# JialeTao/MRFA

Measured on AMD Instinct MI355X. Metric: frames/sec (256x256 source+driving pair) fwd+bwd, higher is better.
Workload: dtype f32; 1 GPU; vox1.yaml MTIA (TokenPose_B) prior + DenseMotion + RaftFlow refinement, 256x256, bs=8/GPU, fwd+bwd+clip+Adam, train-mode BN, surrogate L1 loss; global_batch=8, parallelism=dp1, prior=mtia, background_predictor=False, sync_bn=False, launch=hipGraph, optimizer=FlatAdam (K20), mfma=bf16x6

## Files before the change

mrfa_amd/csrc/common.h:

```cpp
#pragma once
#include <hip/hip_runtime.h>
#include <stdio.h>
#include <string.h>
#include "mrfa_hip.h"

typedef float f32x16 __attribute__((ext_vector_type(16)));
typedef float f32x4 __attribute__((ext_vector_type(4)));

void mrfa_set_error(const char* fmt, ...);

struct MrfaTuning {
    int conv_small_env;
    int conv_small;
    int conv_halo, conv_halo_min_tiles, conv_halo_pr, conv_halo_phase, conv_halo_bn256, conv_halo_bn192, conv_halo_bn64_fill;
    int conv_lean, conv_lean_min_wgs, conv_lean_geo, gemm_lean;
    int wgrad_halo, wgrad_halo_min_wgs, wgrad_halo_target_wgs, wgrad_halo_phase, wgrad_lean;
    int conv_fewout3, attention_mfma, split_target_256;
};
extern MrfaTuning g_tune;

struct HaloGeo { int PR, BN; bool phase; };

enum class ConvFamily { lean, gemm_lean, small, halo, halo_dgrad, rows_split, rows_f32, refused };
struct ConvPlan {
    ConvFamily family;
    char error[256];
    long long M;
    int KT;
    int lean_geo, gemm_cfg, small_tm, small_tn;
    HaloGeo halo;
    int BM, BN, splitk;
    bool w8;
    bool fused;
    bool fin_in_launch;
    bool reads_w;
    int last_config;
    bool groups_ok, bst_ok, stride2_ok, mask_ok, phase_dgrad_ok;
};
ConvPlan plan_conv(const mrfa_conv_params& p);

enum class WgradFamily { lean, small, halo, tiled, refused };
struct WgradPlan {
    WgradFamily family;
    char error[192];
    long long M;
    bool lean, small;
    bool groups_ok, stride2_ok;
};
WgradPlan plan_wgrad(const mrfa_wgrad_params& p);

int mrfa_conv_split_launch(hipStream_t st, const mrfa_conv_params& p, int KT, long long M, int splitk, int BN);
bool mrfa_conv_halo_eligible(const mrfa_conv_params& p, HaloGeo* geo);
int mrfa_conv_halo_launch(hipStream_t st, const mrfa_conv_params& p, const HaloGeo& geo);
int mrfa_wgrad_split_launch(hipStream_t st, const mrfa_wgrad_params& p, dim3 grid, long long M, long long kps, int tiles_n, int nsplit, int inner,
                            int total_splits, int taps, long long partial_stride, int BM, int BN);

bool mrfa_wgrad_halo_eligible(const mrfa_wgrad_params& p);
int mrfa_wgrad_halo_launch(hipStream_t st, const mrfa_wgrad_params& p);

bool mrfa_fewout3_wgrad(hipStream_t st, const float* x, int ldx, int N, int H, int W, int Cin, const float* dy, int lddy, int Cout, int R, int pad,
                        float* dw, float* dbias, int* rc);

int mrfa_conv_lean_pick(const mrfa_conv_params& p);
int mrfa_conv_lean_launch(hipStream_t st, const mrfa_conv_params& p, int geo);
int mrfa_gemm_lean_pick(const mrfa_conv_params& p, long long M);
int mrfa_gemm_lean_launch(hipStream_t st, const mrfa_conv_params& p, long long M, int cfg);

bool mrfa_conv_small_eligible(const mrfa_conv_params& p, long long M);
int mrfa_conv_small_launch(hipStream_t st, const mrfa_conv_params& p, long long M, int tm, int tn);

// ... 137 lines not shown
```

mrfa_amd/csrc/conv_plan.hip:

```cpp
#include "common.h"
#include <stdarg.h>
#include <stdlib.h>

namespace {
int env_int(const char* name, int dflt) { const char* e = getenv(name); return e ? atoi(e) : dflt; }
int env_on(const char* name) { const char* e = getenv(name); return !(e && e[0] == '0'); }
}

MrfaTuning g_tune = {
     env_on("MRFA_CONV_SMALL"),  1,
     env_on("MRFA_CONV_HALO"),  128,  0,  1,  1,
     1,  1,
     env_on("MRFA_CONV_LEAN"),  128,  -1,
     env_int("MRFA_GEMM_LEAN", 1),
     env_on("MRFA_WGRAD_HALO"),  192,  256,  1,
     env_on("MRFA_WGRAD_LEAN"),
     1,  env_on("MRFA_ATTENTION_MFMA"),  env_int("MRFA_SPLIT_TARGET_256", 1),
};

enum TuneKind { T_ON, T_INT, T_NONNEG, T_NONNEG_ON, T_LEVEL, T_POS };
static const struct { const char* key; int* field; TuneKind kind; } TUNING_KEYS[] = {
    {"conv_small", &g_tune.conv_small, T_ON},
    {"conv_halo", &g_tune.conv_halo, T_ON},
    {"conv_halo_min_tiles", &g_tune.conv_halo_min_tiles, T_INT},
    {"conv_halo_pr", &g_tune.conv_halo_pr, T_INT},
    {"conv_halo_phase", &g_tune.conv_halo_phase, T_ON},
    {"conv_halo_bn256", &g_tune.conv_halo_bn256, T_ON},
    {"conv_halo_bn192", &g_tune.conv_halo_bn192, T_ON},
    {"conv_halo_bn64_fill", &g_tune.conv_halo_bn64_fill, T_ON},
    {"conv_lean", &g_tune.conv_lean, T_ON},
    {"conv_lean_min_wgs", &g_tune.conv_lean_min_wgs, T_NONNEG},
    {"conv_lean_geo", &g_tune.conv_lean_geo, T_INT},
    {"gemm_lean", &g_tune.gemm_lean, T_LEVEL},
    {"wgrad_halo", &g_tune.wgrad_halo, T_ON},
    {"wgrad_halo_min_wgs", &g_tune.wgrad_halo_min_wgs, T_NONNEG},
    {"wgrad_halo_target_wgs", &g_tune.wgrad_halo_target_wgs, T_POS},
    {"wgrad_halo_phase", &g_tune.wgrad_halo_phase, T_NONNEG_ON},
    {"wgrad_lean", &g_tune.wgrad_lean, T_ON},
    {"conv_fewout3", &g_tune.conv_fewout3, T_ON},
    {"attention_mfma", &g_tune.attention_mfma, T_ON},
};

extern "C" int mrfa_set_tuning(const char* key, int value) {
    if (!key) return -1;
    for (const auto& k : TUNING_KEYS) {
        if (strcmp(key, k.key)) continue;
        const int prev = *k.field;
        switch (k.kind) {
            case T_ON: *k.field = value != 0; break;
            case T_INT: *k.field = value; break;
            case T_NONNEG: if (value >= 0) *k.field = value; break;
            case T_NONNEG_ON: if (value >= 0) *k.field = value != 0; break;
            case T_LEVEL: if (value >= 0) *k.field = value > 2 ? 2 : value; break;
            case T_POS: if (value > 0) *k.field = value; break;
        }
        return prev;
    }
    return -1;
}

namespace {
constexpr int BK = 32;

template <typename Plan>
Plan& refuse(Plan& c, const char* fmt, ...) {
    va_list ap;
    va_start(ap, fmt);
    vsnprintf(c.error, sizeof(c.error), fmt, ap);
    va_end(ap);
    c.family = decltype(c.family)::refused;
    return c;
}

void plan_rows(ConvPlan& c, const mrfa_conv_params& p, int mode) {
    const bool flat = p.kflat > 0;
    const long long M = c.M;
    const int KT = c.KT;
    const int nb = p.nbatch > 1 ? p.nbatch : 1;
    int BN = 128;
    {
        const int cands[4] = {128, 96, 64, 32};
        const double pen[4] = {1.0, 1.08, 1.16, 1.3};
        double best = 1e18;
        for (int i = 0; i < 4; ++i) {
            if (cands[i] == 96 && flat) continue;
            const double cost = (double)cdiv(p.Cout, cands[i]) * cands[i] * pen[i];
            if (cost < best) { best = cost; BN = cands[i]; }
        }
    }
    if (mode >= 1 && !flat && p.Cout >= 32) BN = p.Cout <= 64 ? 64 : 128;
    auto ntiles = [&](int bm, int bn) { return ((M + bm - 1) / bm) * cdiv(p.Cout, bn) * nb; };
    int BM = 128;
    if (BN == 96 && ntiles(128, 96) < 384) BN = 128;
// ... 164 lines not shown
```

mrfa_amd/csrc/sample.hip:

```cpp
#include "mfma_bf16.h"

namespace {

struct Taps {
    int x0, y0;
    float fx, fy;
};

__device__ __forceinline__ Taps make_taps(float ix, float iy) {
    Taps t;
    const float fx0 = floorf(ix), fy0 = floorf(iy);
    t.x0 = (int)fx0;
    t.y0 = (int)fy0;
    t.fx = ix - fx0;
    t.fy = iy - fy0;
    return t;
}


struct Taps4 {
    size_t o00, o01, o10, o11;
    float w00, w01, w10, w11;
    float fx, fy;
    bool ok00, ok01, ok10, ok11;
// ... 291 lines not shown
__global__ void resize_bwd_kernel(const float* __restrict__ dout, int lddo, int N, int Hi, int Wi, int C, float* __restrict__ din,
                                  int lddi, int Ho, int Wo, float mul, long long total) {
    for (long long i = blockIdx.x * (long long)blockDim.x + threadIdx.x; i < total; i += (long long)gridDim.x * blockDim.x) {
        const long long opix = i / C;
        const int c = (int)(i - opix * C);
        const int ox = (int)(opix % Wo);
        const long long t = opix / Wo;
        const int oy = (int)(t % Ho);
        const long long n = t / Ho;
        int x0, x1, y0, y1;
        float fx, fy;
        resize_src(ox, Wi, Wo, x0, x1, fx);
        resize_src(oy, Hi, Ho, y0, y1, fy);
        const float g = dout[(size_t)opix * lddo + c] * mul;
        float* b = din + (size_t)n * Hi * Wi * lddi + c;
        atomicAdd(b + ((size_t)y0 * Wi + x0) * lddi, g * (1.f - fx) * (1.f - fy));
        atomicAdd(b + ((size_t)y0 * Wi + x1) * lddi, g * fx * (1.f - fy));
        atomicAdd(b + ((size_t)y1 * Wi + x0) * lddi, g * (1.f - fx) * fy);
        atomicAdd(b + ((size_t)y1 * Wi + x1) * lddi, g * fx * fy);
    }
}

__global__ void resize_bwd_gather_kernel(const float* __restrict__ dout, int lddo, int N, int Hi, int Wi, int C, float* __restrict__ din,
                                         int lddi, int Ho, int Wo, float mul, long long total) {
    const float sy = Ho > 1 ? (float)(Hi - 1) / (float)(Ho - 1) : 0.f, sx = Wo > 1 ? (float)(Wi - 1) / (float)(Wo - 1) : 0.f;
    for (long long i = blockIdx.x * (long long)blockDim.x + threadIdx.x; i < total; i += (long long)gridDim.x * blockDim.x) {
        const long long ipix = i / C;
        const int c = (int)(i - ipix * C);
        const int ix = (int)(ipix % Wi);
        const long long t = ipix / Wi;
        const int iy = (int)(t % Hi);
        const long long n = t / Hi;
        int oy_lo = sy > 0.f ? (int)floorf((float)(iy - 1) / sy) - 1 : 0, oy_hi = sy > 0.f ? (int)ceilf((float)(iy + 1) / sy) + 1 : Ho - 1;
        int ox_lo = sx > 0.f ? (int)floorf((float)(ix - 1) / sx) - 1 : 0, ox_hi = sx > 0.f ? (int)ceilf((float)(ix + 1) / sx) + 1 : Wo - 1;
        oy_lo = max(oy_lo, 0); oy_hi = min(oy_hi, Ho - 1); ox_lo = max(ox_lo, 0); ox_hi = min(ox_hi, Wo - 1);
        const float* g = dout + (size_t)n * Ho * Wo * lddo + c;
        float acc = 0.f;
        for (int oy = oy_lo; oy <= oy_hi; ++oy) {
            int y0, y1; float fy;
            resize_src(oy, Hi, Ho, y0, y1, fy);
            const float wy = (y0 == iy ? 1.f - fy : 0.f) + (y1 == iy ? fy : 0.f);
            if (wy == 0.f) continue;
            float row = 0.f;
            for (int ox = ox_lo; ox <= ox_hi; ++ox) {
                int x0, x1; float fx;
                resize_src(ox, Wi, Wo, x0, x1, fx);
                const float wx = (x0 == ix ? 1.f - fx : 0.f) + (x1 == ix ? fx : 0.f);
                if (wx != 0.f) row += wx * g[((size_t)oy * Wo + ox) * lddo];
            }
            acc += wy * row;
        }
        din[(size_t)ipix * lddi + c] += acc * mul;
    }
}

struct ResizeSumArgs {
    int n;
    int prefix[MRFA_RESIZE_SUM_MAX + 1];
    mrfa_resize_sum_desc d[MRFA_RESIZE_SUM_MAX];
};

template <bool BWD>
__global__ __launch_bounds__(256) void resize_sum_multi_kernel(const ResizeSumArgs a) {
    int lo = 0, hi = a.n;
    while (hi - lo > 1) {
        const int mid = (lo + hi) >> 1;
        if ((int)blockIdx.x >= a.prefix[mid]) lo = mid; else hi = mid;
    }
    const mrfa_resize_sum_desc& d = a.d[lo];
    const long long i = (long long)((int)blockIdx.x - a.prefix[lo]) * 256 + threadIdx.x;
    const long long total = (long long)d.N * d.Hd * d.Wd * d.C;
    if (i >= total) return;
    const long long pix = i / d.C;
    const int c = (int)(i - pix * d.C);
    const int px = (int)(pix % d.Wd);
    const long long t = pix / d.Wd;
    const int py = (int)(t % d.Hd);
    const long long n = t / d.Hd;
    float* dst = d.dst + (size_t)pix * d.ldd + c;
    float v = d.overwrite ? 0.f : *dst;
    bool first = d.overwrite != 0;
    for (int k = 0; k < d.nterm; ++k) {
        const float* __restrict__ src = d.term[k].src;
        const int lds = d.term[k].lds, Hs = d.term[k].Hs, Ws = d.term[k].Ws;
        const float mul = d.term[k].mul;
        float r;
        if (Hs == d.Hd && Ws == d.Wd) {
            r = src[(size_t)pix * lds + c] * mul;
        } else if (!BWD) {
            int x0, x1, y0, y1;
            float fx, fy;
            resize_src(px, Ws, d.Wd, x0, x1, fx);
            resize_src(py, Hs, d.Hd, y0, y1, fy);
            const float* b = src + (size_t)n * Hs * Ws * lds + c;
            const float top = b[((size_t)y0 * Ws + x0) * lds] * (1.f - fx) + b[((size_t)y0 * Ws + x1) * lds] * fx;
            const float bot = b[((size_t)y1 * Ws + x0) * lds] * (1.f - fx) + b[((size_t)y1 * Ws + x1) * lds] * fx;
            r = (top * (1.f - fy) + bot * fy) * mul;
        } else {
            const int Hi = d.Hd, Wi = d.Wd, Ho = Hs, Wo = Ws;
            const float sy = Ho > 1 ? (float)(Hi - 1) / (float)(Ho - 1) : 0.f, sx = Wo > 1 ? (float)(Wi - 1) / (float)(Wo - 1) : 0.f;
            int oy_lo = sy > 0.f ? (int)floorf((float)(py - 1) / sy) - 1 : 0, oy_hi = sy > 0.f ? (int)ceilf((float)(py + 1) / sy) + 1 : Ho - 1;
            int ox_lo = sx > 0.f ? (int)floorf((float)(px - 1) / sx) - 1 : 0, ox_hi = sx > 0.f ? (int)ceilf((float)(px + 1) / sx) + 1 : Wo - 1;
            oy_lo = max(oy_lo, 0); oy_hi = min(oy_hi, Ho - 1); ox_lo = max(ox_lo, 0); ox_hi = min(ox_hi, Wo - 1);
            const float* g = src + (size_t)n * Ho * Wo * lds + c;
            float acc = 0.f;
            for (int oy = oy_lo; oy <= oy_hi; ++oy) {
// ... 218 lines not shown
                       in_rep, Hi, Wi, C, grid, ldg, N, Ho, Wo, out, ldo, mode, total);
    MRFA_CHECK_LAUNCH("grid_sample_fwd");
    return 0;
}

extern "C" int mrfa_grid_sample_bf16_fwd(void* stream, const unsigned short* in, int ldi, long long in_bstride, int in_rep, int Hi, int Wi, int C,
                                         const float* grid, int ldg, int N, int Ho, int Wo, float* out, int ldo, int mode) {
    MRFA_CHECK_ARG(in && grid && out && C > 0 && N > 0 && in_rep >= 1 && Hi > 0 && Wi > 0 && Ho > 0 && Wo > 0 && ldi >= C && ldo >= C && ldg >= 2 &&
                   (mode == 0 || mode == 1), "grid_sample_bf16_fwd: bad args");
    MRFA_CHECK_ARG(C % 8 == 0 && ldi % 8 == 0 && in_bstride % 8 == 0 && ldo % 4 == 0 && aligned16(in) && aligned16(out),
                   "grid_sample_bf16_fwd: needs C %% 8 == 0, ldi %% 8 == 0, in_bstride %% 8 == 0, ldo %% 4 == 0 and 16-byte aligned in / out "
                   "(C %d, ldi %d, ldo %d)", C, ldi, ldo);
    const long long npix = (long long)N * Ho * Wo;
    const int c8 = C / 8;
    const int lpp = c8 % 64 == 0 ? 64 : (c8 == 32 ? 32 : (c8 == 16 ? 16 : (c8 == 8 ? 8 : 1)));
    dim3 g(stream_grid(npix * c8, 256));
#define GSH(L) hipLaunchKernelGGL((grid_sample_bf16_fwd_kernel<L>), g, dim3(256), 0, (hipStream_t)stream, in, ldi, in_bstride, in_rep, Hi, Wi, C, \
                                   grid, ldg, npix, Ho, Wo, out, ldo, mode)
    if (lpp == 64) GSH(64); else if (lpp == 32) GSH(32); else if (lpp == 16) GSH(16); else if (lpp == 8) GSH(8); else GSH(1);
#undef GSH
    MRFA_CHECK_LAUNCH("grid_sample_bf16_fwd");
    return 0;
}

extern "C" int mrfa_grid_sample_bwd(void* stream, const float* in, int ldi, long long in_bstride, int in_rep, int Hi, int Wi, int C,
                                    const float* grid, int ldg, int N, int Ho, int Wo, const float* dout, int lddo, int mode,
                                    float* din, int lddi, long long din_bstride, float* dgrid, int lddg) {
    MRFA_CHECK_ARG(in && grid && dout && C > 0 && N > 0 && in_rep >= 1 && Hi > 0 && Wi > 0 && Ho > 0 && Wo > 0 && ldi >= C && lddo >= C && ldg >= 2 &&
                   (!din || lddi >= C) && (!dgrid || lddg >= 2) && (mode == 0 || mode == 1),
                   "grid_sample_bwd: bad args (sizes must be positive, ldi >= C, lddo >= C, ldg >= 2, lddi >= C with din, lddg >= 2 with dgrid, mode 0 or 1; "
                   "C %d, ldi %d, lddo %d, ldg %d, lddi %d, lddg %d, mode %d)", C, ldi, lddo, ldg, lddi, lddg, mode);
    const long long npix = (long long)N * Ho * Wo;
    const int lpp = C % 256 == 0 ? 64 : (C == 128 ? 32 : (C == 64 ? 16 : 0));
    if (lpp && !din && ldi % 4 == 0 && lddo % 4 == 0 && in_bstride % 4 == 0 && aligned16(in) && aligned16(dout)) {
        dim3 g(stream_grid(npix * C / 4, 256));
#define GSB(L) hipLaunchKernelGGL((grid_sample_bwd_vec_kernel<L>), g, dim3(256), 0, (hipStream_t)stream, in, ldi, in_bstride, in_rep, Hi, Wi, C, \
                                   grid, ldg, npix, Ho, Wo, dout, lddo, mode, din, lddi, din_bstride, dgrid, lddg)
        if (lpp == 64) GSB(64); else if (lpp == 32) GSB(32); else GSB(16);
#undef GSB
        MRFA_CHECK_LAUNCH("grid_sample_bwd(vec)");
        return 0;
    }
    const long long waves = (long long)N * Ho * cdiv(Wo, GS_RUN) * cdiv(C, 64);
    hipLaunchKernelGGL(grid_sample_bwd_kernel, dim3(stream_grid(waves * 64, 256)), dim3(256), 0, (hipStream_t)stream, in, ldi, in_bstride,
                       in_rep, Hi, Wi, C, grid, ldg, npix, Ho, Wo, dout, lddo, mode, din, lddi, din_bstride, dgrid, lddg);
    MRFA_CHECK_LAUNCH("grid_sample_bwd");
    return 0;
}

extern "C" int mrfa_resize_bilinear_fwd(void* stream, const float* in, int ldi, int N, int Hi, int Wi, int C, float* out, int ldo,
                                        int Ho, int Wo, float scale_mul, int accumulate) {
    MRFA_CHECK_ARG(in && out && C > 0 && N > 0 && Hi > 0 && Wi > 0 && Ho > 0 && Wo > 0 && ldi >= C && ldo >= C,
                   "resize_fwd: bad args (sizes must be positive, ldi >= C, ldo >= C; C %d, ldi %d, ldo %d, %d x %d -> %d x %d)", C, ldi, ldo, Hi, Wi, Ho, Wo);
    const long long total = (long long)N * Ho * Wo * C;
    hipLaunchKernelGGL(resize_fwd_kernel, dim3(stream_grid(total, 256)), dim3(256), 0, (hipStream_t)stream, in, ldi, N, Hi, Wi, C, out, ldo,
                       Ho, Wo, scale_mul, accumulate, total);
    MRFA_CHECK_LAUNCH("resize_fwd");
    return 0;
}

extern "C" int mrfa_resize_bilinear_bwd(void* stream, const float* dout, int lddo, int N, int Hi, int Wi, int C, float* din, int lddi,
                                        int Ho, int Wo, float scale_mul) {
    MRFA_CHECK_ARG(dout && din && C > 0 && N > 0 && Hi > 0 && Wi > 0 && Ho > 0 && Wo > 0 && lddo >= C && lddi >= C,
                   "resize_bwd: bad args (sizes must be positive, lddo >= C, lddi >= C; C %d, lddo %d, lddi %d, %d x %d -> %d x %d)", C, lddo, lddi, Hi, Wi, Ho, Wo);
    if (Ho >= Hi && Wo >= Wi) {
        const long long total_in = (long long)N * Hi * Wi * C;
        hipLaunchKernelGGL(resize_bwd_gather_kernel, dim3(stream_grid(total_in, 256)), dim3(256), 0, (hipStream_t)stream, dout, lddo, N, Hi,
                           Wi, C, din, lddi, Ho, Wo, scale_mul, total_in);
        MRFA_CHECK_LAUNCH("resize_bwd_gather");
        return 0;
    }
    const long long total = (long long)N * Ho * Wo * C;
    hipLaunchKernelGGL(resize_bwd_kernel, dim3(stream_grid(total, 256)), dim3(256), 0, (hipStream_t)stream, dout, lddo, N, Hi, Wi, C, din,
                       lddi, Ho, Wo, scale_mul, total);
    MRFA_CHECK_LAUNCH("resize_bwd");
    return 0;
}

static int resize_sum_launch(void* stream, const mrfa_resize_sum_desc* descs, int n, bool bwd, const char* what) {
    MRFA_CHECK_ARG(n >= 0 && (n == 0 || descs), "%s: bad args", what);
    for (int base = 0; base < n; base += MRFA_RESIZE_SUM_MAX) {
        ResizeSumArgs a;
        a.n = n - base < MRFA_RESIZE_SUM_MAX ? n - base : MRFA_RESIZE_SUM_MAX;
        int blocks = 0;
        for (int i = 0; i < a.n; ++i) {
            const mrfa_resize_sum_desc& d = descs[base + i];
            MRFA_CHECK_ARG(d.dst && d.N > 0 && d.Hd > 0 && d.Wd > 0 && d.C > 0 && d.nterm >= 1 && d.nterm <= MRFA_RESIZE_SUM_TERMS, "%s: record %d: bad sizes / term count", what, base + i);
            for (int k = 0; k < d.nterm; ++k) {
                MRFA_CHECK_ARG(d.term[k].src && d.term[k].Hs > 0 && d.term[k].Ws > 0, "%s: record %d term %d: null source / bad size", what, base + i, k);
                if (bwd) MRFA_CHECK_ARG(d.term[k].Hs >= d.Hd && d.term[k].Ws >= d.Wd, "%s: record %d term %d: the backward takes up-sampling (or same-size) terms only", what, base + i, k);
            }
            a.d[i] = d;
            a.prefix[i] = blocks;
            const long long total = (long long)d.N * d.Hd * d.Wd * d.C;
            MRFA_CHECK_ARG(total < (1ll << 31) - 256 && blocks + (total + 255) / 256 < (1ll << 30), "%s: record %d too large", what, base + i);
            blocks += (int)((total + 255) / 256);
        }
        a.prefix[a.n] = blocks;
        if (bwd) hipLaunchKernelGGL((resize_sum_multi_kernel<true>), dim3(blocks), dim3(256), 0, (hipStream_t)stream, a);
        else hipLaunchKernelGGL((resize_sum_multi_kernel<false>), dim3(blocks), dim3(256), 0, (hipStream_t)stream, a);
        MRFA_CHECK_LAUNCH(what);
    }
    return 0;
}

extern "C" int mrfa_resize_sum_multi(void* stream, const mrfa_resize_sum_desc* descs, int n) {
    return resize_sum_launch(stream, descs, n, false, "resize_sum_multi");
}

extern "C" int mrfa_resize_sum_multi_bwd(void* stream, const mrfa_resize_sum_desc* descs, int n) {
    return resize_sum_launch(stream, descs, n, true, "resize_sum_multi_bwd");
}

extern "C" int mrfa_corr_lookup_fwd(void* stream, const float* vol0, const float* vol1, int Hs, int Ws, const float* coords, int ldc,
                                    long long Q, int radius, float* out, int ldo) {
    MRFA_CHECK_ARG(radius >= 0 && radius <= 3, "corr_lookup: window must fit one wave (0 <= radius <= 3, got %d)", radius);
    MRFA_CHECK_ARG(vol0 && vol1 && coords && out && Q > 0 && Hs >= 2 && Ws >= 2 && ldc >= 2 && ldo >= 2 * (2 * radius + 1) * (2 * radius + 1),
                   "corr_lookup_fwd: bad args (Hs, Ws >= 2, ldc >= 2, ldo >= 2 (2r+1)^2; Hs %d, Ws %d, ldc %d, ldo %d, radius %d)", Hs, Ws, ldc, ldo, radius);
// ... 57 lines not shown
```

mrfa_amd/engine.py:

```python
from __future__ import annotations

import contextlib
import os

import ctypes as C
from typing import Callable, List, NamedTuple, Optional, Sequence

import torch

from . import hip

BN_EPS = 1e-5
FORCE_TILE = 0
BN_MOMENTUM = 0.1
CAPTURE_KEY = 0
DIRECT_PARAM_GRADS = False
WGRAD_STREAM = False


class Marks:

    def __init__(self, dev, n: int = 256):
        self.buf = torch.zeros(n, dtype=torch.int64, device=dev)
        self.names: List[str] = []
# ... 206 lines not shown

STAT_GROUPS = 1
METRICS_TILE = (32, 32)


class FrameTile(NamedTuple):
    src: torch.Tensor
    y0: int = 0
    x0: int = 0
    kp: Optional[torch.Tensor] = None
    radius: float = 0.0
    colors: Optional[torch.Tensor] = None
    border: bool = False


class stat_groups:

    def __init__(self, groups: int):
        self.groups = int(groups)

    def __enter__(self):
        global STAT_GROUPS
        self.prev, STAT_GROUPS = STAT_GROUPS, self.groups

    def __exit__(self, *exc):
        global STAT_GROUPS
        STAT_GROUPS = self.prev
        return False


class direct_param_grads:
    def __enter__(self):
        global DIRECT_PARAM_GRADS
        self.prev, DIRECT_PARAM_GRADS = DIRECT_PARAM_GRADS, True

    def __exit__(self, *exc):
        global DIRECT_PARAM_GRADS
        DIRECT_PARAM_GRADS = self.prev


def _direct_ok(*params) -> bool:
    return DIRECT_PARAM_GRADS and all(p is None or (p.grad is not None and p.grad.is_contiguous() and p.grad.dtype == torch.float32)
                                      for p in params)


def _r4(c: int) -> int:
    return (c + 3) // 4 * 4


def _up(c: int, m: int) -> int:
    return (c + m - 1) // m * m


def _conv_params() -> hip.ConvParams:
    p = hip.ConvParams()
    p.tile = FORCE_TILE
    return p


class Storage:
    __slots__ = ("data", "dtype", "grad", "rows", "ld", "grad_noinit", "fresh", "bwd_masked", "bn_hint", "seq", "plan")

    def __init__(self, data: torch.Tensor):
        assert data.dim() == 2 and data.dtype in (torch.float32, torch.bfloat16) and data.is_contiguous()
        self.data = data
        self.dtype = data.dtype
        self.rows, self.ld = data.shape
        self.grad: Optional[torch.Tensor] = None
        self.grad_noinit = False
        self.fresh = False
        self.bwd_masked = False
        self.bn_hint = None
        self.seq = -1
        self.plan = None

    def grad_buf(self) -> torch.Tensor:
        if self.dtype != torch.float32:
            raise TypeError("a bf16 storage has no gradient buffer (bf16 activations are inference caches)")
        if self.grad is None:
            self.grad = torch.zeros_like(self.data)
        elif self.fresh:
            self.grad.zero_()
            self.fresh = False
            if self.plan is not None and self.seq >= 0:
                self.plan.add(self.seq)
        return self.grad


class View:
    __slots__ = ("st", "N", "H", "W", "C", "coff", "zpad")

    def __init__(self, st: Storage, N: int, H: int, W: int, C_: int, coff: int = 0, zpad: bool = False):
        assert N * H * W == st.rows and coff + C_ <= st.ld, (N, H, W, C_, coff, st.rows, st.ld)
        self.st, self.N, self.H, self.W, self.C, self.coff = st, N, H, W, C_, coff
        self.zpad = zpad

    @property
    def rows(self) -> int:
        return self.st.rows

    @property
    def ld(self) -> int:
        return self.st.ld

    @property
    def dtype(self) -> torch.dtype:
# ... 478 lines not shown

    def _register(self, st: "Storage"):
        st.seq, st.plan = len(self.storages), self.zero_plan
        self.storages.append(st)

    def wrap_nhwc(self, t: torch.Tensor) -> View:
        assert t.dim() == 4 and t.is_contiguous() and t.dtype == torch.float32
        N, H, W, C_ = t.shape
        return View(Storage(t.view(N * H * W, C_)), N, H, W, C_)

    def from_nchw(self, t: torch.Tensor, out: Optional[View] = None) -> View:
        N, C_, H, W = t.shape
        t = t.contiguous().float()
        out = out or self.new(N, H, W, C_)
        self._chk(self.L.mrfa_nchw_to_nhwc(self.s, t.data_ptr(), out.ptr, out.ld, N, C_, H, W, 0), "nchw_to_nhwc")
        return out

    def to_nchw(self, v: View) -> torch.Tensor:
        t = torch.empty((v.N, v.C, v.H, v.W), dtype=torch.float32, device=self.dev)
        self._chk(self.L.mrfa_nhwc_to_nchw(self.s, v.ptr, v.ld, t.data_ptr(), v.N, v.C, v.H, v.W, 0), "nhwc_to_nchw")
        return t

    def to_bf16(self, v: View) -> View:
        if self.record:
            raise RuntimeError("Ctx.to_bf16: bf16 activations are inference caches, not legal in a recording (training) program")
        out = View(Storage(torch.empty((v.rows, v.C), dtype=torch.bfloat16, device=self.dev)), v.N, v.H, v.W, v.C)
        self._chk(self.L.mrfa_cast_bf16(self.s, v.ptr, v.ld, v.rows, v.C, out.ptr16, out.ld), "cast_bf16")
        return out

    def grad_to_nchw(self, v: View) -> torch.Tensor:
        t = torch.empty((v.N, v.C, v.H, v.W), dtype=torch.float32, device=self.dev)
        self._chk(self.L.mrfa_nhwc_to_nchw(self.s, v.gptr, v.ld, t.data_ptr(), v.N, v.C, v.H, v.W, 0), "nhwc_to_nchw(grad)")
        return t

    def seed_grad_nchw(self, v: View, g: torch.Tensor):
        g = g.contiguous().float()
        self._chk(self.L.mrfa_nchw_to_nhwc(self.s, g.data_ptr(), v.gptr, v.ld, v.N, v.C, v.H, v.W, 1), "seed grad")

    def f32(self, n, zero=False):
        return (torch.zeros if zero else torch.empty)(n, dtype=torch.float32, device=self.dev)

    def f64z(self, n):
        return self.pool64.take(n)

    @staticmethod
    def _claim(v: View) -> bool:
        st = v.st
        if st.grad is not None and st.fresh and v.coff == 0 and v.C == st.ld:
            st.fresh = False
            return True
        return False

    def conv(self, x: View, conv: torch.nn.Conv2d, out: Optional[View] = None, *, relu=False, ups=False, pre=None,
             stats: Optional[torch.Tensor] = None, res: Optional[View] = None, need_dx=True, use_bias=True, relu_in=False, fin=None) -> View:
        cw = convw(conv)
        relu_in = bool(relu_in and RELU_IN and self.record and need_dx and pre is None and not ups)
        if relu_in:
            assert x.coff == 0 and x.C == x.st.ld, "relu_in: the view must cover its storage (every producer skips its ReLU backward)"
            x.st.bwd_masked = True
        assert x.C == cw.Cin, (x.C, cw.Cin)
        Hv, Wv = (x.H * 2, x.W * 2) if ups else (x.H, x.W)
        Ho, Wo = Hv + 2 * cw.pad - cw.R + 1, Wv + 2 * cw.pad - cw.S + 1
        assert out is None or (out.N, out.H, out.W, out.C) == (x.N, Ho, Wo, cw.Cout)
        bias = conv.bias if use_bias else None
        direct = (cw.fewout and not ups and pre is None and res is None and stats is None and not relu
                  and x.ld % 4 == 0 and x.coff % 4 == 0)
        if direct:
            out = out or self.new(x.N, Ho, Wo, cw.Cout)
            self._chk(self.L.mrfa_conv_fewout_fwd(self.s, x.ptr, x.ld, x.N, x.H, x.W, cw.Cin, cw.layout("fewout").data_ptr(),
                                                  bias.data_ptr() if bias is not None else None, out.ptr, out.ld, cw.Cout, cw.R, cw.pad, 0),
                      "conv_fewout_fwd")
            if self.record:
                def bwd_direct():
                    if not out.has_grad:
                        return
                    dw, db = cw.grad_acc(self.pool32)
                    dyp = out.gptr

                    def launch():
                        self._chk(self.L.mrfa_conv_fewout_wgrad(hip.stream_ptr(), x.ptr, x.ld, x.N, x.H, x.W, cw.Cin, dyp, out.ld, cw.Cout, cw.R,
                                                                cw.pad, dw.data_ptr(), db.data_ptr() if (bias is not None and db is not None) else None),
                                  "conv_fewout_wgrad")
                    if self._defer_ok(cw):
                        self.wdefer.add(launch)
                    else:
                        launch()
                    if need_dx:
                        self._conv_dgrad(x, cw, out, ups, pre, relu_in)
                self.tape.append(bwd_direct)
                self._touch(cw)
            return out
        p = _conv_params()
        p.x, p.ldx, p.Hin, p.Win, p.ups, p.N, p.Cin = x.ptr, x.ld, x.H, x.W, int(ups), x.N, cw.Cin
        padded = cw.fwd_flat and x.zpad and x.coff % 4 == 0 and pre is None
        fp32 = self._weight_fields(p, cw, "fwd", padded)
        if self.split and not cw.fwd_flat and ups and cw.R == 3 and cw.S == 3 and cw.pad == 1 and PHASE_UPCONV:
            wph = cw.layout("fwd_phase")
            p.w_phase, p.w_phase_piece = wph.data_ptr(), wph.numel() // 3
        p.Cout, p.Hout, p.Wout = cw.Cout, Ho, Wo
        p.R, p.S, p.pad = cw.R, cw.S, cw.pad
        if pre is not None:
            p.in_scale, p.in_shift, p.in_relu = pre[0].data_ptr(), pre[1].data_ptr(), 1
            if self.train and self.groups > 1:
                p.groups = self.groups
        p.bias = bias.data_ptr() if bias is not None else None
        p.relu = int(relu)
        if res is not None:
            p.res, p.ldr = res.ptr, res.ld
        p.alpha, p.nbatch = 1.0, 1
        if stats is not None:
            p.stats, p.groups = stats.data_ptr(), self.groups
        out = self._conv_out(p, out, x.N, Ho, Wo, cw.Cout)
        late_stats = self._stats_or_late(p, stats, fin, out.rows, pre)
        self._fp32_weights(p, fp32)
        self._launch_conv(p, "conv2d", cw.Cin)
        if late_stats:
            self._bn_stats_into(out, stats)

        if self.record:
            def bwd():
                if not out.has_grad:
                    return
                if relu and not out.st.bwd_masked:
                    self._chk(self.L.mrfa_act_bwd(self.s, out.ptr, out.ld, out.gptr, out.ld, out.rows, out.C, 1, out.gptr, out.ld, 0),
                              "relu_bwd")
                if res is not None:
                    self._chk(self.L.mrfa_copy_view(self.s, out.gptr, out.ld, out.rows, out.C, res.gptr, res.ld, 1.0, 1), "res_bwd")
                if conv.weight.requires_grad:
                    self._conv_wgrad(x, cw, out, ups, pre, bias is not None)
                if need_dx:
                    self._conv_dgrad(x, cw, out, ups, pre, relu_in)
            self.tape.append(bwd)
            self._touch(cw)
        return out

    def _weight_fields(self, p, cw: ConvW, gemm: str, padded: bool = False, planes: bool = True, query: Optional[int] = None):
        g = cw.gemms[gemm]
        rows, k32 = _up(g.rows, 128), _up(g.K, 32)
        if g.flat and not padded:
            p.w_ld, p.w_tap, p.kflat = _up(cw.T * g.K, 32), 0, cw.T * g.K
            p.ktab = g.ktab().data_ptr()
        else:
            p.Cin = k32
            p.w_ld, p.w_tap, p.kflat = k32, rows * k32, 0
            if planes and (self.split or self.bf16):
                p.w_piece = 0 if self.bf16 else cw.T * rows * k32
                p.w_split = query or cw.layout(gemm + ("_rne" if self.bf16 else "_split")).data_ptr()
        p.w_rows = rows
        fp32 = lambda: cw.layout(gemm, padded)
        p.w = query or p.w_split or fp32().data_ptr()
        return fp32

    def _stats_or_late(self, p, stats, fin, rows: int, pre=None) -> bool:
        if stats is None:
            return False
        if self.groups > 1 and not self.L.mrfa_conv2d_groups_supported(C.byref(p)):
            assert pre is None, "a prologue with statistic groups where the library has none: ask prologue_ok() first"
            p.stats, p.groups = None, 0
            return True
        if fin is not None:
            self._fin_params(p, fin, stats, rows)
        return False

    @staticmethod
    def _wgrad_params(x: View, cw: ConvW, dy: int, ldy: int, Ho: int, Wo: int, dw: int, ups=False, stride: int = 0, pre=None) -> hip.WgradParams:
        q = hip.WgradParams()
        q.x, q.ldx, q.Hin, q.Win, q.ups, q.N, q.Cin = x.ptr, x.ld, x.H, x.W, int(ups), x.N, cw.Cin
        if pre is not None:
            q.in_scale, q.in_shift, q.in_relu, q.groups = pre[0], pre[1], 1, pre[2]
        q.dy, q.ldy, q.Cout, q.Hout, q.Wout = dy, ldy, cw.Cout, Ho, Wo
        q.R, q.S, q.pad, q.stride = cw.R, cw.S, cw.pad, stride
        q.dw, q.alpha, q.nbatch, q.ksplit = dw, 1.0, 1, 0
        return q

    def _fp32_weights(self, p, pack):
        ph = p.w_split or p.w_phase
        if not ph or p.w != ph:
            return
        if not (LAZY_FP32_PACKS and not self.L.mrfa_conv2d_reads_fp32_weights(C.byref(p))):
            p.w = pack().data_ptr()

    def _conv_out(self, p, out: Optional[View], N, Ho, Wo, Cout) -> View:
        rows = N * Ho * Wo
        if FUSED_SPLITK and rows <= 32768:
# ... 1213 lines not shown
```

mrfa_amd/modules/raft.py:

```python
from __future__ import annotations

import functools
import math
from typing import List

import torch
import torch.nn.functional as F
from torch import nn

from ..engine import Ctx, Storage, View, run_program
from .generator import OcclusionAwareGenerator
from .util import _FN, Hourglass, batch_bilinear_sampler, bilinear_sampler, coords_grid, coords_grid_nhwc, kp2gaussian


class CorrBlock:

    def __init__(self, corr, num_levels=2, radius=3):
        if num_levels != 2:
            raise NotImplementedError("CorrBlock: the lookup kernel holds the reference's two pyramid levels (raft.py:238)")
        assert corr.dim() == 4 and corr.shape[1] == 1 and corr.shape[2] % 2 == 0 and corr.shape[3] % 2 == 0
        self.num_levels, self.radius = num_levels, radius
        self.corr = corr

    def __call__(self, coords):
        corr, r = self.corr, self.radius
        BQ, _, H, W = corr.shape
        B, _, h1, w1 = coords.shape
        assert B * h1 * w1 == BQ, "CorrBlock: one source map per query pixel"

        def program(e: Ctx, corr_, coords_):
            vol0 = corr_.contiguous().float().view(BQ, H * W)
            vol1 = torch.empty((BQ, (H // 2) * (W // 2)), dtype=torch.float32, device=vol0.device)
            e._chk(e.L.mrfa_avgpool2_fwd(e.s, vol0.data_ptr(), 1, BQ, H, W, 1, vol1.data_ptr(), 1), "corr pyramid level 1")
            cv = e.wrap_nhwc(coords_.float().permute(0, 2, 3, 1).contiguous())
            d = {}

            def dvols():
                if not d:
                    d[0], d[1] = torch.zeros_like(vol0), torch.zeros_like(vol1)
                return d[0], d[1]
            o = e.corr_lookup(vol0, vol1, dvols, H, W, cv, radius=r)

            def dcorr():
                if not d:
                    return None
                e._chk(e.L.mrfa_unpool2_acc(e.s, d[1].data_ptr(), 1, BQ, H // 2, W // 2, 1, d[0].data_ptr(), 1, 0.25), "corr pyramid bwd")
                return d[0].view(BQ, 1, H, W)
            return (e.to_nchw(o),), (lambda g: e.seed_grad_nchw(o, g),), \
                (dcorr, (lambda: cv.st.grad.view(B, h1, w1, 2).permute(0, 3, 1, 2) if cv.has_grad else None))
        return run_program(_FN, program, [corr, coords])[0]


class BasicMotionEncoder(nn.Module):

    def __init__(self, num_levels=2, radius=3):
        super().__init__()
        cor_planes = num_levels * (2 * radius + 1) ** 2
        self.convc1 = nn.Conv2d(cor_planes, 128, 1, padding=0)
        self.convc2 = nn.Conv2d(128, 96, 3, padding=1)
        self.convf1 = nn.Conv2d(2, 128, 7, padding=3)
        self.convf2 = nn.Conv2d(128, 64, 3, padding=1)
        self.conv = nn.Conv2d(64 + 96, 128 - 2, 3, padding=1)

    def run(self, e: Ctx, flow: View, corr: View, out: View):
        cor1 = e.conv(corr, self.convc1, relu=True)
        corflo = e.new(flow.N, flow.H, flow.W, 160)
        e.conv(cor1, self.convc2, out=corflo.slice(0, 96), relu=True, relu_in=True)
        flo1 = e.conv(flow, self.convf1, relu=True)
        e.conv(flo1, self.convf2, out=corflo.slice(96, 160), relu=True, relu_in=True)
        e.conv(corflo, self.conv, out=out.slice(0, 126), relu=True, relu_in=True)
        e.copy(flow, out=out.slice(126, 128))

    def forward(self, delta_flow, corr):
        def program(e: Ctx, flow_, corr_):
            fv = e.from_nchw(flow_)
            cv = e.from_nchw(corr_, out=e.new(corr_.shape[0], corr_.shape[2], corr_.shape[3], corr_.shape[1], pad32=True))
            out = e.new(fv.N, fv.H, fv.W, 128)
            self.run(e, fv, cv, out)
            return (e.to_nchw(out),), (lambda g: e.seed_grad_nchw(out, g),), \
                ((lambda: e.grad_to_nchw(fv) if fv.has_grad else None), (lambda: e.grad_to_nchw(cv) if cv.has_grad else None))
        return run_program(self, program, [delta_flow, corr])[0]


class RefineFlow(nn.Module):

    def __init__(self):
        super().__init__()
        self.convc1 = nn.Conv2d(192, 128, 3, padding=1)
        self.conv1 = nn.Conv2d(256, 128, 3, padding=1)
        self.conv2 = nn.Conv2d(128, 2, 3, padding=1)
        self.convo1 = nn.Conv2d(256, 128, 3, padding=1)
        self.convo2 = nn.Conv2d(128, 1, 3, padding=1)

    def run(self, e: Ctx, inp: View, ctx: View, ctx_relu=False) -> View:
        e.conv(ctx, self.convc1, out=inp.slice(128, 256), relu=True, relu_in=ctx_relu)
        h1 = e.conv(inp, self.conv1, relu=True)
        d = e.new(inp.N, inp.H, inp.W, 3)
        e.conv(h1, self.conv2, out=d.slice(0, 2), relu_in=True)
        h2 = e.conv(inp, self.convo1, relu=True)
        e.conv(h2, self.convo2, out=d.slice(2, 3), relu_in=True)
        return d

    def forward(self, m_f, warp_f):
        def program(e: Ctx, mf_, wf_):
            inp = e.new(mf_.shape[0], mf_.shape[2], mf_.shape[3], 256)
            mv = e.from_nchw(mf_, out=inp.slice(0, 128))
            wv = e.from_nchw(wf_)
            d = self.run(e, inp, wv)
            return (e.to_nchw(d), e.to_nchw(inp)), ((lambda g: e.seed_grad_nchw(d, g)), (lambda g: e.seed_grad_nchw(inp, g))), \
                ((lambda: e.grad_to_nchw(mv) if mv.has_grad else None), (lambda: e.grad_to_nchw(wv) if wv.has_grad else None))
        out, inp = run_program(self, program, [m_f, warp_f])
        return out, inp


class _CorrVolume:

    def __init__(self, e: Ctx, q: View, k: View, kpool: View, scale: float):
        self.e, self.q, self.k, self.kp, self.scale = e, q, k, kpool, scale
        B, Q, S0, S1, D = q.N, q.H * q.W, k.H * k.W, kpool.H * kpool.W, q.C
        self.B, self.Q, self.S0, self.S1, self.D = B, Q, S0, S1, D
        Bs = k.N
        T = B // Bs
        assert Bs * T == B and kpool.N == Bs, "_CorrVolume: the frames of every source, consecutive"
        if T > 1 and e.record:
# ... 139 lines not shown
            outs = (e.to_nchw(out), e.to_nchw(warp_img), self._strip(e, occs))
            seed = ((lambda g: e.seed_grad_nchw(out, g)), (lambda g: e.seed_grad_nchw(warp_img, g)), None)
            return outs, seed, in_grads

        pos = self.pos_embedding

        in_d = e.kp_gaussian(kp_d, 0.1, e.new(b, h, w, kp_d.shape[1]), pos=pos)
        if cache is not None:
            k_s, k_pool = cache["k_s"], cache["k_pool"]
            fe_d = self.kp.run(e, in_d)
            q_d = e.conv(fe_d, self.kp_head)
        else:
            in_s = self._source_input(e, kp_s, img, h, w)
            k_s = e.conv(self.kp_img.run(e, in_s), self.kp_img_head)
            k_pool = e.avgpool2(k_s)
            fe_d = self.kp.run(e, in_d)
            q_d = e.conv(fe_d, self.kp_head)
        in_grads = ((lambda: e.ext_grads.get(id(kp_s))), (lambda: e.ext_grads.get(id(kp_d)))) + in_grads[2:]
        base = self.basic_res_index
        q_levels = {base: q_d}
        for i in range(base - 1, -1, -1):
            q_levels[i] = e.avgpool2(q_levels[i + 1])
        vols = {i: _CorrVolume(e, q_levels[i], k_s, k_pool, self.scale) for i in range(base + 1)} if corr == "volume" else None

        with e.fused_resizes():
            init_flow = e.copy(deform, mul=(h - 1) / 2.0)
            e.copy(_grid_const(e, b, h, w, -1.0, (h - 1) / 2.0, img_full), out=init_flow, acc=True, nograd=True)
        r0 = size // 32
        with e.fused_resizes():
            flow = e.resize(init_flow, r0, r0, mul=1.0 / 8.0)
            occ = e.resize(prior_occ, r0, r0)

        lv_c = gen.level_channels()
        cats = [e.new(b, r0 * (2 ** i), r0 * (2 ** i), 2 * lv_c[i]) for i in range(gen.num_up_blocks)]

        out_warp_f, out_occ = [], []
        d_f_pre = d_occ_pre = None
        for i in range(self.total_iter):
            r = r0 * (2 ** i)
            f = feature[i]
            if i < base:
                cscale, lv, rq = float(2 ** (base - i)), i, r
                flow_q = flow
            else:
                cscale, lv, rq = 1.0, base, h
                flow_q = e.resize(flow, h, w, mul=0.5 ** (i - base)) if i > base else flow
            with e.fused_resizes():
                coords = e.copy(flow_q, mul=cscale)
                e.copy(_grid_const(e, b, rq, rq, cscale, 0.0, img_full), out=coords, acc=True, nograd=True)
            if vols is not None:
                cfeat = e.corr_lookup(vols[lv].vol0, vols[lv].vol1, vols[lv].dvols, h, w, coords)
            else:
                cfeat = e.corr_direct(q_levels[lv], k_s, k_pool, coords, self.scale, k_rep=T)
            if i > base:
                cfeat = e.resize(cfeat, r, r)
            inp = e.new(b, r, r, 256)
            self.corr_enc.run(e, flow, cfeat, inp)
            ctx = e.grid_sample(f, flow, 1, in_rep=T)
            ctx = e.conv(ctx, self.to_context[i], relu=True)
            d_flow = self.refine.run(e, inp, ctx, ctx_relu=True)
            grid_c = None
            with e.fused_resizes():
                flow_w = e.copy(flow)
                e.copy(d_flow.slice(0, 2), out=flow_w, acc=True)
                occ_new = e.copy(occ)
                e.copy(d_flow.slice(2, 3), out=occ_new, acc=True)
                if i < gen.num_up_blocks:
                    grid_c = e.resize(deform, r, r) if i != base else deform
                if i < self.num_iter - 1:
                    r2 = r * 2
                    sc = 2 ** (base - i) / 2.0
                    nflow = e.resize(d_flow.slice(0, 2), r2, r2, mul=2.0)
                    e.resize(init_flow, r2, r2, mul=1.0 / sc, out=nflow, acc=True)
                    nocc = e.resize(d_flow.slice(2, 3), r2, r2)
                    e.resize(prior_occ, r2, r2, out=nocc, acc=True)
                    if i == 0:
                        d_f_pre = e.resize(d_flow.slice(0, 2), r2, r2, mul=2.0)
                        d_occ_pre = e.resize(d_flow.slice(2, 3), r2, r2)
                    else:
                        e.resize(d_f_pre, r2, r2, mul=2.0, out=nflow, acc=True)
                        e.resize(d_occ_pre, r2, r2, out=nocc, acc=True)
                        nd = e.resize(d_flow.slice(0, 2), r2, r2, mul=2.0)
                        e.resize(d_f_pre, r2, r2, mul=2.0, out=nd, acc=True)
                        no = e.resize(d_flow.slice(2, 3), r2, r2)
                        e.resize(d_occ_pre, r2, r2, out=no, acc=True)
                        d_f_pre, d_occ_pre = nd, no
            out_warp_f.append(e.grid_sample(f, flow_w, 1, in_rep=T))
            out_occ.append(e.act(occ_new, 2))
            if i < gen.num_up_blocks:
                e.grid_sample(f, grid_c, 0, out=cats[i].slice(lv_c[i], 2 * lv_c[i]), in_rep=T)
            if i < self.num_iter - 1:
                flow, occ = nflow, nocc
        warp_img = e.grid_sample(imgf, flow, 1, in_rep=T, need_din=False)
        out = gen.run_decode(e, out_warp_f, warp_img, out_occ, cats)
        strip = self._strip(e, out_occ + [e.act(prior_occ, 2)])
        outs = (e.to_nchw(out), e.to_nchw(warp_img), strip)
        seed = ((lambda g: e.seed_grad_nchw(out, g)), (lambda g: e.seed_grad_nchw(warp_img, g)), None)
        return outs, seed, in_grads

    def forward(self, kp_s, kp_d, dense_motion, img, img_full, source_cache=None, corr="volume"):
        if check_corr(corr) == "direct":
            if self.training:
                raise ValueError('corr="direct" is an inference mode (the direct correlation kernel has no backward): call eval() first, training keeps the volumes')
            ins_grad = (kp_s, kp_d, dense_motion['deformation'], dense_motion['occlusion'])
            if torch.is_grad_enabled() and any(t.requires_grad for t in (*self.parameters(), *ins_grad)):
                raise ValueError('corr="direct" has no backward: run it under torch.no_grad() (gradients are enabled and a parameter or input requires one)')
        bs = source_cache["shape"][0] if source_cache is not None else img_full.shape[0]
        b = dense_motion['deformation'].shape[0]
        if b != bs:
            if source_cache is None:
# ... 18 lines not shown
```

Baseline: 101.8 pairs/s.

## Apply 1x1 corr conv before upsampling and add vectorized resize kernels

For refinement levels above base, the 1x1 convc1 now runs on the low-resolution correlation features and its pre-activation output is bilinearly upsampled, with the ReLU applied as a prologue of convc2. Because both the 1x1 conv and bilinear resize are linear, this commutes and cuts the 1x1 conv work and the resize channel count. Separately, float4-vectorized resize forward and gather-backward kernels are added behind a tuning flag. The risks are that the bias now passes through the resize (bilinear weights sum to one, so it is preserved), the ReLU prologue path uses identity scale/shift vectors, and the backward masking must be handled through the new relu_pro flag.

```diff
diff --git a/mrfa_amd/csrc/common.h b/mrfa_amd/csrc/common.h
--- a/mrfa_amd/csrc/common.h
+++ b/mrfa_amd/csrc/common.h
@@ -16,6 +16,7 @@
     int conv_lean, conv_lean_min_wgs, conv_lean_geo, gemm_lean;
     int wgrad_halo, wgrad_halo_min_wgs, wgrad_halo_target_wgs, wgrad_halo_phase, wgrad_lean;
     int conv_fewout3, attention_mfma, split_target_256;
+    int resize_vec;
 };
 extern MrfaTuning g_tune;
 
diff --git a/mrfa_amd/csrc/conv_plan.hip b/mrfa_amd/csrc/conv_plan.hip
--- a/mrfa_amd/csrc/conv_plan.hip
+++ b/mrfa_amd/csrc/conv_plan.hip
@@ -16,6 +16,7 @@
      env_on("MRFA_WGRAD_HALO"),  192,  256,  1,
      env_on("MRFA_WGRAD_LEAN"),
      1,  env_on("MRFA_ATTENTION_MFMA"),  env_int("MRFA_SPLIT_TARGET_256", 1),
+     1,
 };
 
 enum TuneKind { T_ON, T_INT, T_NONNEG, T_NONNEG_ON, T_LEVEL, T_POS };
@@ -39,6 +40,7 @@
     {"wgrad_lean", &g_tune.wgrad_lean, T_ON},
     {"conv_fewout3", &g_tune.conv_fewout3, T_ON},
     {"attention_mfma", &g_tune.attention_mfma, T_ON},
+    {"resize_vec", &g_tune.resize_vec, T_ON},
 };
 
 extern "C" int mrfa_set_tuning(const char* key, int value) {
diff --git a/mrfa_amd/csrc/sample.hip b/mrfa_amd/csrc/sample.hip
--- a/mrfa_amd/csrc/sample.hip
+++ b/mrfa_amd/csrc/sample.hip
@@ -367,6 +367,108 @@
         }
         din[(size_t)ipix * lddi + c] += acc * mul;
     }
+}
+
+struct ResizeVecGeo { int lg, C4, cpr, units; };
+
+__global__ __launch_bounds__(256) void resize_fwd_vec_kernel(const float* __restrict__ in, int ldi, int Hi, int Wi, float* __restrict__ out, int ldo,
+                                                             int Ho, int Wo, float mul, int acc, ResizeVecGeo g) {
+    for (int u = blockIdx.x; u < g.units; u += gridDim.x) {
+        const int row = u / g.cpr;
+        const int j = (u - row * g.cpr) * 256 + (int)threadIdx.x;
+        const int ox = j >> g.lg, q = j & ((1 << g.lg) - 1);
+        if (ox >= Wo || q >= g.C4) continue;
+        const int n = row / Ho, oy = row - n * Ho;
+        int x0, x1, y0, y1;
+        float fx, fy;
+        resize_src(ox, Wi, Wo, x0, x1, fx);
+        resize_src(oy, Hi, Ho, y0, y1, fy);
+        const float* b = in + (size_t)n * Hi * Wi * ldi + 4 * q;
+        const f32x4 v00 = *(const f32x4*)(b + ((size_t)y0 * Wi + x0) * ldi), v01 = *(const f32x4*)(b + ((size_t)y0 * Wi + x1) * ldi);
+        const f32x4 v10 = *(const f32x4*)(b + ((size_t)y1 * Wi + x0) * ldi), v11 = *(const f32x4*)(b + ((size_t)y1 * Wi + x1) * ldi);
+        f32x4* d = (f32x4*)(out + ((size_t)row * Wo + ox) * ldo + 4 * q);
+        f32x4 r = acc ? *d : f32x4{0.f, 0.f, 0.f, 0.f};
+#pragma unroll
+        for (int k = 0; k < 4; ++k) {
+            const float top = v00[k] * (1.f - fx) + v01[k] * fx;
+            const float bot = v10[k] * (1.f - fx) + v11[k] * fx;
+            const float v = (top * (1.f - fy) + bot * fy) * mul;
+            r[k] = acc ? (r[k] + v) : v;
+        }
+        *d = r;
+    }
+}
+
+__device__ __forceinline__ float resize_tap_weight(int o, int i, int Ni, int No) {
+    int i0, i1; float f;
+    resize_src(o, Ni, No, i0, i1, f);
+    return (i0 == i ? 1.f - f : 0.f) + (i1 == i ? f : 0.f);
+}
+__device__ __forceinline__ void resize_tap_range(int i, int Ni, int No, int& lo, int& hi) {
+    const float s = No > 1 ? (float)(Ni - 1) / (float)(No - 1) : 0.f;
+    lo = s > 0.f ? (int)floorf((float)(i - 1) / s) - 1 : 0;
+    hi = s > 0.f ? (int)ceilf((float)(i + 1) / s) + 1 : No - 1;
+    lo = max(lo, 0); hi = min(hi, No - 1);
+    while (lo <= hi && resize_tap_weight(lo, i, Ni, No) == 0.f) ++lo;
+    while (hi >= lo && resize_tap_weight(hi, i, Ni, No) == 0.f) --hi;
+}
+
+__global__ __launch_bounds__(256) void resize_bwd_gather_vec_kernel(const float* __restrict__ dout, int lddo, int Hi, int Wi, float* __restrict__ din,
+                                                                    int lddi, int Ho, int Wo, float mul, ResizeVecGeo g) {
+    for (int u = blockIdx.x; u < g.units; u += gridDim.x) {
+        const int row = u / g.cpr;
+        const int j = (u - row * g.cpr) * 256 + (int)threadIdx.x;
+        const int ix = j >> g.lg, q = j & ((1 << g.lg) - 1);
+        if (ix >= Wi || q >= g.C4) continue;
+        const int n = row / Hi, iy = row - n * Hi;
+        int oy_lo, oy_hi, ox_lo, ox_hi;
+        resize_tap_range(iy, Hi, Ho, oy_lo, oy_hi);
+        resize_tap_range(ix, Wi, Wo, ox_lo, ox_hi);
+        const float* gp = dout + (size_t)n * Ho * Wo * lddo + 4 * q;
+        f32x4 acc = {0.f, 0.f, 0.f, 0.f};
+        for (int oy = oy_lo; oy <= oy_hi; ++oy) {
+            const float wy = resize_tap_weight(oy, iy, Hi, Ho);
+            if (wy == 0.f) continue;
+            const float* gr = gp + (size_t)oy * Wo * lddo;
+            f32x4 rsum = {0.f, 0.f, 0.f, 0.f};
+            for (int ox0 = ox_lo; ox0 <= ox_hi; ox0 += 8) {
+                f32x4 v[8];
+                float wx[8];
+#pragma unroll
+                for (int t = 0; t < 8; ++t) {
+                    const int ox = min(ox0 + t, ox_hi);
+                    v[t] = *(const f32x4*)(gr + (size_t)ox * lddo);
+                    wx[t] = ox0 + t <= ox_hi ? resize_tap_weight(ox, ix, Wi, Wo) : 0.f;
+                }
+#pragma unroll
+                for (int t = 0; t < 8; ++t) {
+                    if (wx[t] != 0.f) {
+#pragma unroll
+                        for (int k = 0; k < 4; ++k) rsum[k] += wx[t] * v[t][k];
+                    }
+                }
+            }
+#pragma unroll
+            for (int k = 0; k < 4; ++k) acc[k] += wy * rsum[k];
+        }
+        f32x4* d = (f32x4*)(din + ((size_t)row * Wi + ix) * lddi + 4 * q);
+        f32x4 r = *d;
+#pragma unroll
+        for (int k = 0; k < 4; ++k) r[k] += acc[k] * mul;
+        *d = r;
+    }
+}
+
+static bool resize_vec_geo(const void* a, int lda, const void* b, int ldb, long long rows, int W, int C, ResizeVecGeo& g) {
+    if (!g_tune.resize_vec || C % 4 || lda % 4 || ldb % 4 || (((uintptr_t)a | (uintptr_t)b) & 15)) return false;
+    g.C4 = C / 4;
+    g.lg = 0;
+    while ((1 << g.lg) < g.C4) ++g.lg;
+    const long long lanes = (long long)W << g.lg, cpr = (lanes + 255) / 256;
+    if (lanes >= (1ll << 30) || rows * cpr >= (1ll << 30)) return false;
+    g.cpr = (int)cpr;
+    g.units = (int)(rows * cpr);
+    return true;
 }
 
 struct ResizeSumArgs {
@@ -691,6 +793,13 @@
                                         int Ho, int Wo, float scale_mul, int accumulate) {
     MRFA_CHECK_ARG(in && out && C > 0 && N > 0 && Hi > 0 && Wi > 0 && Ho > 0 && Wo > 0 && ldi >= C && ldo >= C,
                    "resize_fwd: bad args (sizes must be positive, ldi >= C, ldo >= C; C %d, ldi %d, ldo %d, %d x %d -> %d x %d)", C, ldi, ldo, Hi, Wi, Ho, Wo);
+    ResizeVecGeo vg;
+    if (resize_vec_geo(in, ldi, out, ldo, (long long)N * Ho, Wo, C, vg)) {
+        hipLaunchKernelGGL(resize_fwd_vec_kernel, dim3(vg.units < 256 * 16 ? vg.units : 256 * 16), dim3(256), 0, (hipStream_t)stream, in, ldi, Hi, Wi,
+                           out, ldo, Ho, Wo, scale_mul, accumulate, vg);
+        MRFA_CHECK_LAUNCH("resize_fwd_vec");
+        return 0;
+    }
     const long long total = (long long)N * Ho * Wo * C;
     hipLaunchKernelGGL(resize_fwd_kernel, dim3(stream_grid(total, 256)), dim3(256), 0, (hipStream_t)stream, in, ldi, N, Hi, Wi, C, out, ldo,
                        Ho, Wo, scale_mul, accumulate, total);
@@ -703,6 +812,13 @@
     MRFA_CHECK_ARG(dout && din && C > 0 && N > 0 && Hi > 0 && Wi > 0 && Ho > 0 && Wo > 0 && lddo >= C && lddi >= C,
                    "resize_bwd: bad args (sizes must be positive, lddo >= C, lddi >= C; C %d, lddo %d, lddi %d, %d x %d -> %d x %d)", C, lddo, lddi, Hi, Wi, Ho, Wo);
     if (Ho >= Hi && Wo >= Wi) {
+        ResizeVecGeo vg;
+        if (resize_vec_geo(dout, lddo, din, lddi, (long long)N * Hi, Wi, C, vg)) {
+            hipLaunchKernelGGL(resize_bwd_gather_vec_kernel, dim3(vg.units < 256 * 16 ? vg.units : 256 * 16), dim3(256), 0, (hipStream_t)stream, dout,
+                               lddo, Hi, Wi, din, lddi, Ho, Wo, scale_mul, vg);
+            MRFA_CHECK_LAUNCH("resize_bwd_gather_vec");
+            return 0;
+        }
         const long long total_in = (long long)N * Hi * Wi * C;
         hipLaunchKernelGGL(resize_bwd_gather_kernel, dim3(stream_grid(total_in, 256)), dim3(256), 0, (hipStream_t)stream, dout, lddo, N, Hi,
                            Wi, C, din, lddi, Ho, Wo, scale_mul, total_in);
diff --git a/mrfa_amd/engine.py b/mrfa_amd/engine.py
--- a/mrfa_amd/engine.py
+++ b/mrfa_amd/engine.py
@@ -282,6 +282,19 @@
     return (c + m - 1) // m * m
 
 
+_RELU_PRO_VECS: dict = {}
+
+
+def _relu_pro_vectors(dev: torch.device, c: int):
+    key = (dev, c)
+    v = _RELU_PRO_VECS.get(key)
+    if v is None:
+        v = (torch.ones(c, dtype=torch.float32, device=dev), torch.zeros(c, dtype=torch.float32, device=dev))
+        if not (dev.type == "cuda" and torch.cuda.is_current_stream_capturing()):
+            _RELU_PRO_VECS[key] = v
+    return v
+
+
 def _conv_params() -> hip.ConvParams:
     p = hip.ConvParams()
     p.tile = FORCE_TILE
@@ -866,9 +879,17 @@
         return False
 
     def conv(self, x: View, conv: torch.nn.Conv2d, out: Optional[View] = None, *, relu=False, ups=False, pre=None,
-             stats: Optional[torch.Tensor] = None, res: Optional[View] = None, need_dx=True, use_bias=True, relu_in=False, fin=None) -> View:
+             stats: Optional[torch.Tensor] = None, res: Optional[View] = None, need_dx=True, use_bias=True, relu_in=False, fin=None,
+             relu_pro=False) -> View:
         cw = convw(conv)
+        if relu_pro:
+            assert pre is None and not ups and stats is None and not relu_in, "relu_pro: a plain convolution of relu(x)"
+            ones, zeros = _relu_pro_vectors(x.st.data.device, cw.Cin)
+            pre_w = (ones, zeros, {"groups": 1})
+        else:
+            pre_w = pre
         relu_in = bool(relu_in and RELU_IN and self.record and need_dx and pre is None and not ups)
+        mask_in = relu_in or bool(relu_pro and self.record and need_dx)
         if relu_in:
             assert x.coff == 0 and x.C == x.st.ld, "relu_in: the view must cover its storage (every producer skips its ReLU backward)"
             x.st.bwd_masked = True
@@ -877,7 +898,7 @@
         Ho, Wo = Hv + 2 * cw.pad - cw.R + 1, Wv + 2 * cw.pad - cw.S + 1
         assert out is None or (out.N, out.H, out.W, out.C) == (x.N, Ho, Wo, cw.Cout)
         bias = conv.bias if use_bias else None
-        direct = (cw.fewout and not ups and pre is None and res is None and stats is None and not relu
+        direct = (cw.fewout and not ups and pre is None and res is None and stats is None and not relu and not relu_pro
                   and x.ld % 4 == 0 and x.coff % 4 == 0)
         if direct:
             out = out or self.new(x.N, Ho, Wo, cw.Cout)
@@ -906,7 +927,7 @@
             return out
         p = _conv_params()
         p.x, p.ldx, p.Hin, p.Win, p.ups, p.N, p.Cin = x.ptr, x.ld, x.H, x.W, int(ups), x.N, cw.Cin
-        padded = cw.fwd_flat and x.zpad and x.coff % 4 == 0 and pre is None
+        padded = cw.fwd_flat and x.zpad and x.coff % 4 == 0 and pre is None and not relu_pro
         fp32 = self._weight_fields(p, cw, "fwd", padded)
         if self.split and not cw.fwd_flat and ups and cw.R == 3 and cw.S == 3 and cw.pad == 1 and PHASE_UPCONV:
             wph = cw.layout("fwd_phase")
@@ -917,6 +938,8 @@
             p.in_scale, p.in_shift, p.in_relu = pre[0].data_ptr(), pre[1].data_ptr(), 1
             if self.train and self.groups > 1:
                 p.groups = self.groups
+        if relu_pro:
+            p.in_scale, p.in_shift, p.in_relu = ones.data_ptr(), zeros.data_ptr(), 1
         p.bias = bias.data_ptr() if bias is not None else None
         p.relu = int(relu)
         if res is not None:
@@ -941,9 +964,9 @@
                 if res is not None:
                     self._chk(self.L.mrfa_copy_view(self.s, out.gptr, out.ld, out.rows, out.C, res.gptr, res.ld, 1.0, 1), "res_bwd")
                 if conv.weight.requires_grad:
-                    self._conv_wgrad(x, cw, out, ups, pre, bias is not None)
+                    self._conv_wgrad(x, cw, out, ups, pre_w, bias is not None)
                 if need_dx:
-                    self._conv_dgrad(x, cw, out, ups, pre, relu_in)
+                    self._conv_dgrad(x, cw, out, ups, pre, mask_in)
             self.tape.append(bwd)
             self._touch(cw)
         return out
diff --git a/mrfa_amd/modules/raft.py b/mrfa_amd/modules/raft.py
--- a/mrfa_amd/modules/raft.py
+++ b/mrfa_amd/modules/raft.py
@@ -2,6 +2,7 @@
 
 import functools
 import math
+import os
 from typing import List
 
 import torch
@@ -11,6 +12,9 @@
 from ..engine import Ctx, Storage, View, run_program
 from .generator import OcclusionAwareGenerator
 from .util import _FN, Hourglass, batch_bilinear_sampler, bilinear_sampler, coords_grid, coords_grid_nhwc, kp2gaussian
+
+
+CORR_CONV_FIRST = os.environ.get("MRFA_CORR_CONV_FIRST", "1") != "0"
 
 
 class CorrBlock:
@@ -62,14 +66,24 @@
         self.convf2 = nn.Conv2d(128, 64, 3, padding=1)
         self.conv = nn.Conv2d(64 + 96, 128 - 2, 3, padding=1)
 
-    def run(self, e: Ctx, flow: View, corr: View, out: View):
-        cor1 = e.conv(corr, self.convc1, relu=True)
+    def run(self, e: Ctx, flow: View, corr: View, out: View, cor1_pre: View = None):
         corflo = e.new(flow.N, flow.H, flow.W, 160)
-        e.conv(cor1, self.convc2, out=corflo.slice(0, 96), relu=True, relu_in=True)
+        if cor1_pre is not None:
+            e.conv(cor1_pre, self.convc2, out=corflo.slice(0, 96), relu=True, relu_pro=True)
+        else:
+            cor1 = e.conv(corr, self.convc1, relu=True)
+            e.conv(cor1, self.convc2, out=corflo.slice(0, 96), relu=True, relu_in=True)
         flo1 = e.conv(flow, self.convf1, relu=True)
         e.conv(flo1, self.convf2, out=corflo.slice(96, 160), relu=True, relu_in=True)
         e.conv(corflo, self.conv, out=out.slice(0, 126), relu=True, relu_in=True)
         e.copy(flow, out=out.slice(126, 128))
+
+    def run_upsampled(self, e: Ctx, flow: View, cfeat: View, out: View):
+        if CORR_CONV_FIRST:
+            z = e.conv(cfeat, self.convc1)
+            self.run(e, flow, None, out, cor1_pre=e.resize(z, flow.H, flow.W))
+        else:
+            self.run(e, flow, e.resize(cfeat, flow.H, flow.W), out)
 
     def forward(self, delta_flow, corr):
         def program(e: Ctx, flow_, corr_):
@@ -315,10 +329,11 @@
                 cfeat = e.corr_lookup(vols[lv].vol0, vols[lv].vol1, vols[lv].dvols, h, w, coords)
             else:
                 cfeat = e.corr_direct(q_levels[lv], k_s, k_pool, coords, self.scale, k_rep=T)
+            inp = e.new(b, r, r, 256)
             if i > base:
-                cfeat = e.resize(cfeat, r, r)
-            inp = e.new(b, r, r, 256)
-            self.corr_enc.run(e, flow, cfeat, inp)
+                self.corr_enc.run_upsampled(e, flow, cfeat, inp)
+            else:
+                self.corr_enc.run(e, flow, cfeat, inp)
             ctx = e.grid_sample(f, flow, 1, in_rep=T)
             ctx = e.conv(ctx, self.to_context[i], relu=True)
             d_flow = self.refine.run(e, inp, ctx, ctx_relu=True)
```

Result: no change. 101.5 pairs/s (-0.2%).
